# zhangyi-3/UCDIR

Hardware: AMD Instinct MI355X
Metric: restored images/sec at 50-step p_sample_loop, 256x256 SID (higher is better)
Workload: dtype bf16

## Files before the change

### ucdir_amd/csrc/conv_ws128.hip.h

```cpp
#pragma once
#include <type_traits>
#include "conv_ws.hip.h"

struct CvWs128 {
    static constexpr int PITCH = 24;
    static constexpr int PLANE = 10 * PITCH * 128;
    static constexpr int HALO = 2 * PLANE;
    static constexpr int QSTEP = 2 * PITCH * 128;
    static constexpr int OFF_A2 = 2 * HALO;
    static constexpr int A2_BYTES = 2 * 8 * 2 * 32 * 16;
    static constexpr int OFF_TCS = OFF_A2 + A2_BYTES;
    static constexpr int OFF_B2 = OFF_TCS + 9 * 64 * 4;
    static constexpr int OFF_SCAL = OFF_B2 + 64 * 4;
    static constexpr int LDS = OFF_SCAL + 128;
    static constexpr int THREADS = 256;
    static constexpr int DEPTH = 3;
};

__global__ __launch_bounds__(CvWs128::THREADS, 1) void conv_ws128_kernel(const GemmP p) {
    using L = CvWs128;
    extern __shared__ __attribute__((aligned(16))) unsigned char smem[];
    float* const tcs = reinterpret_cast<float*>(smem + L::OFF_TCS);
    float* const b2s = reinterpret_cast<float*>(smem + L::OFF_B2);
    float* const scal = reinterpret_cast<float*>(smem + L::OFF_SCAL);
    const int tid = threadIdx.x, lane = tid & 63, l31 = lane & 31, hh = lane >> 5;
    const int wave = __builtin_amdgcn_readfirstlane(tid >> 6);
    const int rw = wave & 1, pw = wave >> 1;
    const int prow = l31 >> 4, pcol = (l31 & 15) ^ (prow << 3);
    int lid;
    {
        const int nblk = gridDim.x, bid = blockIdx.x;
        const int q = nblk >> 3, r = nblk & 7, xcd = bid & 7;
        lid = (xcd < r ? xcd * (q + 1) : r * (q + 1) + (xcd - r) * q) + (bid >> 3);
    }
#ifdef UCDIR_TIMING
    const bool dbg_on = p.dbg && (lid == (int)gridDim.x / 2 + 3) && (lane == 0) && (wave == 1);
    int dbg_n = 0;
#define C8_STAMP() do { if (dbg_on && dbg_n < 250) p.dbg[dbg_n++] = __builtin_amdgcn_s_memtime(); } while (0)
#else
#define C8_STAMP() do {} while (0)
#endif
    C8_STAMP();
    const int tps = p.tiles_x * p.tiles_y;
    const int T = p.nbatch * tps;
    const int t_beg = (int)((long long)lid * T / (int)gridDim.x), t_end = (int)((long long)(lid + 1) * T / (int)gridDim.x);
    if (t_beg >= t_end) return;

    bf16x8_t af[72];
    {
        const bf16_t* Ab = p.A + ((rw * 72 * 2 + hh) * 32 + l31) * 8;
#pragma unroll
        for (int j = 0; j < 72; ++j) af[j] = *reinterpret_cast<const bf16x8_t*>(Ab + j * (2 * 32 * 8));
    }
#pragma unroll
    for (int j = 0; j < 72; ++j) asm volatile("" : "+v"(af[j]));
    for (int i = tid; i < L::A2_BYTES / 16; i += L::THREADS)
        reinterpret_cast<uint4*>(smem + L::OFF_A2)[i] = reinterpret_cast<const uint4*>(p.alt_A)[i];
    if (tid < 64) b2s[tid] = p.bias2 ? p.bias2[tid] : 0.f;
    __syncthreads();

    unsigned hrel[3];
#pragma unroll
    for (int c3 = 0; c3 < 3; ++c3) {
        const int col = c3 * 8 + (lane >> 3), hp = wave * L::PITCH + col;
        hrel[c3] = col < 18 ? (unsigned)((wave * p.Wp + col) * 64 + (((lane & 7) ^ ((hp >> 1) & 7)) << 3)) * 2u : 0xffffffffu;
    }
    unsigned ba[3][4];
    {
        const int hp0 = (4 * pw + prow) * L::PITCH + pcol;
#pragma unroll
        for (int kx = 0; kx < 3; ++kx) {
            const int sxh = (((hp0 + kx) >> 1) & 7) ^ hh;
#pragma unroll
            for (int k2 = 0; k2 < 4; ++k2) ba[kx][k2] = ((hp0 + kx) << 7) + (((2 * k2) ^ sxh) << 4);
        }
    }
    const unsigned tc_lane = L::OFF_TCS + (32 * rw + 16 * hh) * 4;
    const unsigned b2_lane = L::OFF_B2 + (32 * rw + 16 * hh) * 4;
    const unsigned a2_lane = L::OFF_A2 + ((rw * 8 * 2 + hh) * 32 + l31) * 16;
    const unsigned rel_out = (unsigned)(((4 * pw + prow + 1) * p.Wp + pcol + 1) * 64 + 32 * rw + 16 * hh) * 2;

    int b, ty, tx;
    {
        b = t_beg / tps;
        const int r = t_beg - b * tps;
        ty = r / p.tiles_x; tx = r - ty * p.tiles_x;
    }
    auto issue_tile = [&](int nb, int nty, int ntx, int buf) {
        const long long pix0 = (long long)nty * 8 * p.Wp + ntx * 16;
        const unsigned char* h0 = reinterpret_cast<const unsigned char*>(p.B0 + (long long)nb * p.b0_bstride + pix0 * 64);
        const unsigned char* h1 = reinterpret_cast<const unsigned char*>(p.B1 + (long long)nb * p.b1_bstride + pix0 * 64);
        unsigned char* hd = smem + buf * L::HALO;
        const long long r4 = (long long)4 * p.Wp * 64 * 2;
#pragma unroll
        for (int c3 = 0; c3 < 3; ++c3)
            if (hrel[c3] != 0xffffffffu) {
#pragma unroll
                for (int k = 0; k < 3; ++k)
                    if (k < 2 || wave < 2) {
                        stage16(reinterpret_cast<const bf16_t*>(h0 + k * r4 + hrel[c3]), hd + (3 * (wave + 4 * k) + c3) * 1024, lane);
                        stage16(reinterpret_cast<const bf16_t*>(h1 + k * r4 + hrel[c3]), hd + L::PLANE + (3 * (wave + 4 * k) + c3) * 1024, lane);
                    }
            }
    };
    issue_tile(b, ty, tx, 0);

    int b_cur = -1;
    float rstd_a = 1.f;
    stat_t S1 = 0, S2 = 0;
    const int act = p.act;

#pragma unroll 1
    for (int t = t_beg; t < t_end; ++t) {
        const int buf = (t - t_beg) & 1;
        const bool last = t + 1 == t_end;
        C8_STAMP();
        if (t == t_beg) { HC_WAIT(0); }
        asm volatile("s_barrier" ::: "memory");
        C8_STAMP();
        if (b != b_cur) {
            if (b_cur >= 0 && p.stats_out) {
                const stat_t a = wave_sum_ll(S1), q2 = wave_sum_ll(S2);
                if (lane == 0) stat_add_fx(p.stats_out, b_cur, a, q2);
            }
            S1 = 0; S2 = 0;
            b_cur = b;
            if (wave == 0) {
                float mean = 0.f, rstd = 1.f;
                if (p.fold) {
                    long long v = 0;
                    if (lane < 2 * UCDIR_STAT_SLOTS) {
                        v = p.stats0[(long long)b * (2 * UCDIR_STAT_SLOTS) + lane];
                        if (p.stats1) v += p.stats1[(long long)b * (2 * UCDIR_STAT_SLOTS) + lane];
                    }
#pragma unroll
                    for (int off = 2; off < 2 * UCDIR_STAT_SLOTS; off <<= 1) v += __shfl_xor(v, off);
                    const long long q = __shfl(v, 1);
                    mean_rstd(stat_val(v), stat_val(q), p.inv_count, mean, rstd);
                }
                if (lane == 0) { scal[0] = mean; scal[1] = rstd; }
            }
            __syncthreads();
            const float mean = scal[0], rstd = scal[1];
            for (int i = tid; i < 9 * 64; i += L::THREADS) {
                const int cls = i >> 6, f = i & 63;
                float v = p.bias ? p.bias[f] : 0.f;
                if (p.fold) v += p.Tb[(long long)cls * p.tab_ld + f] - mean * rstd * p.Tg[(long long)cls * p.tab_ld + f];
                tcs[i] = v;
            }
            rstd_a = __builtin_bit_cast(float, __builtin_amdgcn_readfirstlane(__builtin_bit_cast(int, p.alpha * (p.fold ? rstd : 1.0f))));
            __syncthreads();
        }
        int nb = b, nty = ty, ntx = tx + 1;
        if (ntx == p.tiles_x) { ntx = 0; if (++nty == p.tiles_y) { nty = 0; ++nb; } }
        C8_STAMP();

        if (t != t_beg) {
            const int d = buf ? L::HALO : -L::HALO;
#pragma unroll
            for (int kx = 0; kx < 3; ++kx)
#pragma unroll
                for (int k2 = 0; k2 < 4; ++k2) ba[kx][k2] += d;
        }

        f32x16_t acc[2];
        {
            bf16x8_t bq[L::DEPTH + 1][2];
            const long long npix0 = (long long)nty * 8 * p.Wp + ntx * 16;
            const unsigned char* h0 = reinterpret_cast<const unsigned char*>(p.B0 + (long long)nb * p.b0_bstride + npix0 * 64);
            const unsigned char* h1 = reinterpret_cast<const unsigned char*>(p.B1 + (long long)nb * p.b1_bstride + npix0 * 64);
            unsigned char* const hd = smem + (buf ^ 1) * L::HALO;
            const long long r4 = (long long)4 * p.Wp * 64 * 2;
            __builtin_amdgcn_sched_barrier(0);
            asm volatile("s_waitcnt lgkmcnt(0)" ::: "memory");
            static_for<0, L::DEPTH>([&](auto jc) {
                constexpr int j = decltype(jc)::value;
                constexpr int tap = j >> 3, c16 = j & 7, ky = tap / 3, kx = tap - 3 * ky;
                constexpr int off = (c16 >> 2) * L::PLANE + ky * (L::PITCH * 128);
                lds_read16_asm<off>(bq[j][0], ba[kx][(c16 & 3) ^ (ky == 1 ? 2 : 0)]);
                lds_read16_asm<off + L::QSTEP>(bq[j][1], ba[kx][(c16 & 3) ^ (ky == 1 ? 2 : 0)]);
            });
            static_for<0, 72>([&](auto jc) {
                constexpr int j = decltype(jc)::value;
                if constexpr (j + L::DEPTH < 72) {
                    constexpr int jn = j + L::DEPTH;
                    constexpr int tap = jn >> 3, c16 = jn & 7, ky = tap / 3, kx = tap - 3 * ky;
                    constexpr int off = (c16 >> 2) * L::PLANE + ky * (L::PITCH * 128);
                    lds_read16_asm<off>(bq[jn % (L::DEPTH + 1)][0], ba[kx][(c16 & 3) ^ (ky == 1 ? 2 : 0)]);
                    lds_read16_asm<off + L::QSTEP>(bq[jn % (L::DEPTH + 1)][1], ba[kx][(c16 & 3) ^ (ky == 1 ? 2 : 0)]);
                }
                if constexpr (j % 4 == 1 && j / 4 < 18) {
                    constexpr int e = j / 4, c3 = e / 6, k = (e % 6) >> 1, pl = e & 1;
                    if (!last && (k < 2 || wave < 2) && hrel[c3] != 0xffffffffu)
                        stage16(reinterpret_cast<const bf16_t*>((pl ? h1 : h0) + k * r4 + hrel[c3]),
                                hd + pl * L::PLANE + (3 * (wave + 4 * k) + c3) * 1024, lane);
                }
                constexpr int ahead = (71 - j) < L::DEPTH ? (71 - j) : L::DEPTH;
                lgkm_wait_asm<2 * ahead>();
                const f32x16_t zero = {0.f, 0.f, 0.f, 0.f, 0.f, 0.f, 0.f, 0.f, 0.f, 0.f, 0.f, 0.f, 0.f, 0.f, 0.f, 0.f};
                acc[0] = __builtin_amdgcn_mfma_f32_32x32x16_bf16(af[j], bq[j % (L::DEPTH + 1)][0], j ? acc[0] : zero, 0, 0, 0);
                acc[1] = __builtin_amdgcn_mfma_f32_32x32x16_bf16(af[j], bq[j % (L::DEPTH + 1)][1], j ? acc[1] : zero, 0, 0, 0);
            });
            __builtin_amdgcn_sched_barrier(0);
        }
        C8_STAMP();
        f32x16_t acc2[2];
        {
            const f32x16_t zero = {0.f, 0.f, 0.f, 0.f, 0.f, 0.f, 0.f, 0.f, 0.f, 0.f, 0.f, 0.f, 0.f, 0.f, 0.f, 0.f};
#pragma unroll
            for (int j = 0; j < 8; ++j) {
                const bf16x8_t a2 = *reinterpret_cast<const bf16x8_t*>(smem + a2_lane + j * 1024);
                const unsigned a0 = ba[1][(j & 3) ^ 2] + (j >> 2) * L::PLANE + L::PITCH * 128;
                const bf16x8_t b0 = *reinterpret_cast<const bf16x8_t*>(smem + a0);
                const bf16x8_t b1 = *reinterpret_cast<const bf16x8_t*>(smem + a0 + L::QSTEP);
                acc2[0] = __builtin_amdgcn_mfma_f32_32x32x16_bf16(a2, b0, j ? acc2[0] : zero, 0, 0, 0);
                acc2[1] = __builtin_amdgcn_mfma_f32_32x32x16_bf16(a2, b1, j ? acc2[1] : zero, 0, 0, 0);
            }
        }

        C8_STAMP();
        const bool interior = ty > 0 && tx > 0 && ty + 1 < p.tiles_y && tx + 1 < p.tiles_x;
        const long long tile_el = (long long)(ty * 8 * p.Wp + tx * 16) * 64;
        unsigned char* outb = reinterpret_cast<unsigned char*>(reinterpret_cast<bf16_t*>(p.out) + (long long)b * p.out_bstride + tile_el);
        unsigned char* out2b = reinterpret_cast<unsigned char*>(p.out2 + (long long)b * p.out2_bstride + tile_el);
        float s1 = 0.f, s2 = 0.f;
        uint4 pk[2][2], pk2[2][2];
#pragma unroll
        for (int tp = 0; tp < 2; ++tp) {
            unsigned tca = tc_lane + 4 * 256;
            if (!interior) {
                const int r = 4 * pw + 2 * tp + prow, c = pcol;
                const int cy = (ty == 0 && r == 0) ? 0 : ((ty + 1 == p.tiles_y && r == 7) ? 2 : 1);
                const int cx = (tx == 0 && c == 0) ? 0 : ((tx + 1 == p.tiles_x && c == 15) ? 2 : 1);
                tca = tc_lane + (cy * 3 + cx) * 256;
            }
            float v[16], w[16];
#pragma unroll
            for (int g4 = 0; g4 < 4; ++g4) {
                const f32x4_t c4 = *reinterpret_cast<const f32x4_t*>(smem + tca + 16 * g4);
                const f32x4_t d4 = *reinterpret_cast<const f32x4_t*>(smem + b2_lane + 16 * g4);
#pragma unroll
                for (int e = 0; e < 4; ++e) {
                    v[4 * g4 + e] = fmaf(acc[tp][4 * g4 + e], rstd_a, c4[e]);
                    w[4 * g4 + e] = acc2[tp][4 * g4 + e] + d4[e];
                }
            }
            if (act == 1) {
#pragma unroll
                for (int i = 0; i < 16; ++i) v[i] = silu_fast(v[i]);
            } else if (act == 2) {
#pragma unroll
                for (int i = 0; i < 16; ++i) v[i] = fmaxf(0.2f * v[i], v[i]);
            }
#pragma unroll
            for (int i = 0; i < 16; ++i) { s1 += v[i]; s2 += v[i] * v[i]; }
            pk[tp][0] = pack8_bf16(v); pk[tp][1] = pack8_bf16(v + 8);
            pk2[tp][0] = pack8_bf16(w); pk2[tp][1] = pack8_bf16(w + 8);
        }
        C8_STAMP();
        HC_WAIT(0);
        C8_STAMP();
#pragma unroll
        for (int tp = 0; tp < 2; ++tp) {
            const long long o = rel_out + (long long)tp * (2 * p.Wp * 64 * 2);
            *reinterpret_cast<uint4*>(outb + o) = pk[tp][0];
            *reinterpret_cast<uint4*>(outb + o + 16) = pk[tp][1];
            *reinterpret_cast<uint4*>(out2b + o) = pk2[tp][0];
            *reinterpret_cast<uint4*>(out2b + o + 16) = pk2[tp][1];
        }
        S1 += stat_fx((double)s1); S2 += stat_fx((double)s2);
        b = nb; ty = nty; tx = ntx;
    }
#ifdef UCDIR_TIMING
    if (dbg_on) p.dbg[255] = dbg_n;
#endif
    if (p.stats_out) {
        const stat_t a = wave_sum_ll(S1), q2 = wave_sum_ll(S2);
        if (lane == 0) stat_add_fx(p.stats_out, b_cur, a, q2);
    }
}
```

### ucdir_amd/csrc/engine.hip

```cpp
#include <hip/hip_runtime.h>

#include <cmath>
#include <cstdio>
#include <cstring>
#include <map>
#include <mutex>
#include <set>
#include <array>
#include <atomic>
#include <memory>
#include <string>
#include <vector>

#include "../../include/ucdir_hip.h"
#include "cgemm.hip.h"
#include "conv_halo.hip.h"
#include "akgm_halo.hip.h"
#include "akgm_pre.hip.h"
#include "akgm_ws.hip.h"
#include "akgm_ws32.hip.h"
#include "akgm_ws64.hip.h"
#include "conv_ws.hip.h"
#include "conv_sk.hip.h"
#include "conv_ws128.hip.h"
// ... 1244 lines not shown
            fl += 2.0 * 9 * d.cin * d.cout * h * w;
        } else {
            const int h = level_dim(c->Hc, d.level), w = level_dim(c->Wc, d.level);
            if (d.skip_c) { require(!skips.empty(), "skip stack underflow"); x1 = (long)skips.back(); skips.pop_back(); }
            r.h1 = ap.get(h, w, d.cout);
            if (d.cin != d.cout) r.res = ap.get(h, w, d.cout, false);
            r.out = ap.get(h, w, d.cout);
            if (d.attn) r.bo = ap.get(h, w, d.cout);
            r.G = (float*)c->apool.alloc((size_t)B * h * w * 8 * sizeof(float));
            const double hw = (double)h * w;
            fl += 2.0 * 9 * d.cin * d.cout * hw + 2.0 * 9 * d.cout * d.cout * hw;
            if (d.cin != d.cout) fl += 2.0 * d.cin * d.cout * hw;
            fl += 2.0 * hw * (3 * 16 + 72 * 8);
            if (d.attn) {
                if (h * w > maxN) maxN = h * w;
                attC = d.cout;
                fl += 2.0 * d.cout * 3 * d.cout * hw + 2.0 * d.cout * d.cout * hw + 4.0 * hw * hw * d.cout;
            }
            ap.put(r.h1); ap.put(r.res); ap.put(r.bo);
        }
        if (x1 >= 0) ap.put(c->rt[x1].out);
        if (cur >= 0 && !is_skip[cur]) ap.put(c->rt[cur].out);
        cur = (long)li;
        if (d.push_skip) { skips.push_back(li); is_skip[li] = true; }
    }
    fl += 2.0 * 9 * c->cfg.inner_channel * c->cfg.channel_mults[0] * c->cfg.out_channel * c->Hc * c->Wc;
    c->flops = fl * B;
    c->fin_act = Act();
    if (!c->fin_w || env().no_fused_final) c->fin_act = make_act(c->apool, B, c->Hc, c->Wc, c->cfg.inner_channel * c->cfg.channel_mults[0], false);
    if (maxN > 0) alloc_attn(c->apool, c->attn, B, maxN, attC, c->cfg.attn_fp16 != 0);
    c->attw = (float*)c->apool.alloc((size_t)c->nblocks * B * 8 * sizeof(float));
    {
        int maxC = 0;
        for (const auto& d : c->layers) if (d.kind == "block" && d.cout > maxC) maxC = d.cout;
        c->tcbuf = (float*)c->apool.alloc((size_t)B * (9 * 8 * maxC + 2) * sizeof(float), false);
    }
    c->guide_ready = false;
}

static void forward(ucdir_ctx* c, const float* cond, const float* xt, const float* level, float* eps, hipStream_t st) {
    struct ScratchScope { ScratchScope(float* p) { t_splitk = p; } ~ScratchScope() { t_splitk = nullptr; } } scratch_scope(c->splitk);
    c->apool.zero_stats(st);
    require(c->finalized, "weights not finalized");
    require(c->guide_ready, "ucdir_prepare_guide must be called before ucdir_unet_forward");
    const int B = c->B, inner = c->cfg.inner_channel;
    {
        const size_t sm = (size_t)(6 * inner + c->nblocks * 8) * sizeof(float);
        hipLaunchKernelGGL(time_mlp_kernel, dim3(B), dim3(256), sm, st, level, inner, c->mlp_w1, c->mlp_b1, c->mlp_w2,
                           c->mlp_b2, c->tw, c->nblocks, c->attw, B);
        HIPC(hipGetLastError());
    }
    std::vector<const Act*> skips;
    const Act* cur = nullptr;
    for (size_t li = 0; li < c->layers.size(); ++li) {
        const LayerDesc& d = c->layers[li];
        const LayerW& w = c->lw[li];
        LayerRT& r = c->rt[li];
        if (d.kind == "stem") {
            const int tx = (c->Wc + 15) / 16, ty = (c->Hc + 15) / 16;
            const int units = tx * ty * (d.cout / 64) * B;
            hipLaunchKernelGGL((stem_mfma_kernel<6, 0>), dim3(units < 4 * num_cus() ? units : 4 * num_cus()), dim3(256), 0, st, cond, xt, c->H, c->W,
                               c->Hc, c->Wc, d.cout, tx, w.stem_w, r.out.p, r.out.stats, tx * ty, d.cout / 64, B);
            HIPC(hipGetLastError());
        } else if (d.kind == "down") {
            run_conv(w.conv, COLS_DOWN, {*cur, nullptr, r.out, 0, nullptr, true}, st);
        } else if (d.kind == "up") {
            run_conv(w.conv, COLS_UP, {*cur, nullptr, r.out, 0, nullptr, true}, st);
        } else {
            const Act* x0 = cur; const Act* x1 = nullptr;
            if (d.skip_c) { x1 = skips.back(); skips.pop_back(); require(x1->C == d.skip_c, "skip channel mismatch"); }
            const bool res_done = run_conv(w.conv, COLS_S1, {*x0, x1, r.h1, 1, nullptr, true, w.has_res ? &r.res : nullptr, w.has_res ? &w.resconv : nullptr}, st);
            const Act* res = x0;
            if (w.has_res) { if (!res_done) run_conv(w.resconv, COLS_S1, {*x0, x1, r.res, 0, nullptr, false}, st); res = &r.res; }
            Act& bo = d.attn ? r.bo : r.out;
            run_akgm(w.sp, r.h1, r.G, c->attw + (size_t)w.block_index * B * 8, *res, bo, c->tcbuf, st);
            if (d.attn) run_attention(w.qkv, w.outp, bo, r.out, c->attn, st);
        }
        cur = &r.out;
        if (d.push_skip) skips.push_back(cur);
    }
    {
        const int C = cur->C, co = c->cfg.out_channel;
        if (!env().no_fused_final && c->fin_w) {
            const int tiles = ((c->Wc + 15) / 16) * ((c->Hc + 15) / 16) * B;
            const dim3 grid(tiles < 3 * num_cus() ? tiles : 3 * num_cus());
            const size_t lds = (size_t)324 * 80 + (size_t)9 * (C / 32) * 1024 + (size_t)8 * C + (size_t)8 * B;
            require(lds <= 160 * 1024, "final conv: channel count too large for the fused kernel");
            hipLaunchKernelGGL(final_conv_kernel, grid, dim3(256), lds, st, cur->p, c->Hc, c->Wc, C, cur->stats,
                               1.0 / ((double)C * c->Hc * c->Wc), c->fin_gamma, c->fin_beta, c->fin_w, c->fin_b, co, eps, c->H, c->W, B);
            HIPC(hipGetLastError());
        } else {
            hipLaunchKernelGGL(gn_silu_kernel, dim3(2048, 1, B), dim3(256), 0, st, cur->p, c->fin_act.p, c->Hc, c->Wc, C,
                               cur->stats, 1.0 / ((double)C * c->Hc * c->Wc), c->fin_gamma, c->fin_beta);
            HIPC(hipGetLastError());
            Act dummy; dummy.B = B; dummy.H = c->Hc; dummy.W = c->Wc; dummy.C = c->fin_conv.cout;
            run_conv(c->fin_conv, COLS_S1, {c->fin_act, nullptr, dummy, 0, nullptr, false, nullptr, nullptr, eps, c->H, c->W}, st);
        }
    }
}

static void forward_graph(ucdir_ctx* c, const float* cond, const float* xt, const float* level, float* eps, hipStream_t st) {
    for (auto& f : c->graphs)
        if (f.cond == cond && f.xt == xt && f.lvl == level && f.eps == eps) { c->miss_streak = 0; HIPC(hipGraphLaunch(f.ex, st)); return; }
    const bool same_as_last = c->last_miss[0] == cond && c->last_miss[1] == xt && c->last_miss[2] == level && c->last_miss[3] == eps;
    c->last_miss[0] = cond; c->last_miss[1] = xt; c->last_miss[2] = level; c->last_miss[3] = eps;
    if (c->miss_streak >= 2 && !same_as_last) { ++c->miss_streak; forward(c, cond, xt, level, eps, st); return; }
    ++c->miss_streak;
    if (c->graphs.size() >= 8) { const int ms = c->miss_streak; c->drop_graphs(); c->miss_streak = ms; }
    if (!c->cap_stream) HIPC(hipStreamCreateWithFlags(&c->cap_stream, hipStreamNonBlocking));
    HIPC(hipStreamSynchronize(st));
    ucdir_ctx::FwdGraph f{cond, xt, level, eps, nullptr, nullptr};
    HIPC(hipStreamBeginCapture(c->cap_stream, hipStreamCaptureModeThreadLocal));
    try { forward(c, cond, xt, level, eps, c->cap_stream); }
    catch (...) { hipGraph_t g = nullptr; (void)hipStreamEndCapture(c->cap_stream, &g); if (g) (void)hipGraphDestroy(g); throw; }
    HIPC(hipStreamEndCapture(c->cap_stream, &f.g));
    if (hipGraphInstantiate(&f.ex, f.g, nullptr, nullptr, 0) != hipSuccess) {
        (void)hipGraphDestroy(f.g);
        throw std::runtime_error("hipGraphInstantiate failed for a captured forward");
    }
    c->graphs.push_back(f);
    HIPC(hipGraphLaunch(f.ex, st));
}

extern "C" {

int32_t ucdir_abi_version(void) { return UCDIR_ABI_VERSION; }
const char* ucdir_last_error(void) { return g_err.c_str(); }

int32_t ucdir_create(const ucdir_config* cfg, ucdir_ctx** out) {
    API_BEGIN
    require(cfg && out, "null argument");
    require(cfg->n_mults >= 1 && cfg->n_mults <= UCDIR_MAX_MULTS, "bad n_mults");
    require(cfg->inner_channel % 64 == 0, "inner_channel must be a multiple of 64");
    int ndev = 0;
    hipError_t e = hipGetDeviceCount(&ndev);
    require(e == hipSuccess && ndev > 0, "no HIP device available (libucdir_hip has no CPU fallback)");
    require(cfg->device >= 0 && cfg->device < ndev, "bad device ordinal");
    DevGuard dg(cfg->device);
    ensure_kernel_attrs();
    std::unique_ptr<ucdir_ctx> c(new ucdir_ctx());
    c->cfg = *cfg;
    c->layers = build_layers(*cfg);
    for (const auto& d : c->layers)
        if (d.kind == "block") require(d.cout == 64 || d.cout % 128 == 0, "block channels must be 64 or a multiple of 128");
    c->wnames = expected_names(*cfg, c->layers);
    *out = c.release();
    API_END
}

void ucdir_destroy(ucdir_ctx* ctx) {
    if (!ctx) return;
    try { DevGuard dg(ctx->cfg.device); ctx->drop_graphs(); delete ctx; } catch (...) {}
}

int32_t ucdir_num_weights(const ucdir_ctx* ctx) { return ctx ? (int32_t)ctx->wnames.size() : 0; }
const char* ucdir_weight_name(const ucdir_ctx* ctx, int32_t i) {
    if (!ctx || i < 0 || i >= (int32_t)ctx->wnames.size()) return nullptr;
    return ctx->wnames[i].c_str();
}

int32_t ucdir_load_weight(ucdir_ctx* ctx, const char* name, const float* data_host, const int64_t* shape, int32_t ndim) {
    API_BEGIN
    require(ctx && name && data_host && shape, "null argument");
    HostT t; size_t n = 1;
    for (int i = 0; i < ndim; ++i) { t.shape.push_back(shape[i]); n *= (size_t)shape[i]; }
    t.v.assign(data_host, data_host + n);
    ctx->host[name] = std::move(t);
    ctx->finalized = false;
    API_END
// ... 1066 lines not shown
```

### ucdir_amd/csrc/misc.hip.h

```cpp
#pragma once
#include "common.h"

__global__ void act_stats_kernel(const bf16_t* __restrict__ x, int H, int W, int C, stat_t* __restrict__ stats) {
    const int b = blockIdx.x;
    const int Wp = W + 2;
    const long long bs = (long long)(H + 2) * Wp * C;
    const int c8 = C / 8;
    double s1 = 0, s2 = 0;
    for (long long i = threadIdx.x; i < (long long)H * W * c8; i += blockDim.x) {
        int c = (int)(i % c8);
        long long pix = i / c8;
        int y = (int)(pix / W), xx = (int)(pix % W);
        const uint4 v = *reinterpret_cast<const uint4*>(x + b * bs + ((long long)(y + 1) * Wp + xx + 1) * C + c * 8);
        const bf16_t* h = reinterpret_cast<const bf16_t*>(&v);
#pragma unroll
        for (int k = 0; k < 8; ++k) { float f = bf2f(h[k]); s1 += f; s2 += (double)f * f; }
    }
    __shared__ double sh[2][256];
    sh[0][threadIdx.x] = s1; sh[1][threadIdx.x] = s2;
    __syncthreads();
    for (int o = 128; o > 0; o >>= 1) {
        if ((int)threadIdx.x < o) { sh[0][threadIdx.x] += sh[0][threadIdx.x + o]; sh[1][threadIdx.x] += sh[1][threadIdx.x + o]; }
        __syncthreads();
    }
// ... 108 lines not shown
                if (j == 4 && hh) bfr[tp] = __builtin_bit_cast(bf16x8_t, make_uint4(0x3F803F80u, 0u, 0u, 0u));
            }
#pragma unroll
            for (int tm = 0; tm < 2; ++tm)
#pragma unroll
                for (int tp = 0; tp < 2; ++tp)
                    acc[tm][tp] = __builtin_amdgcn_mfma_f32_32x32x16_bf16(af[tm], bfr[tp], acc[tm][tp], 0, 0, 0);
        }
        float s1 = 0.f, s2 = 0.f;
        unsigned char* ot = otile + wv * (32 * 144);
#pragma unroll
        for (int tp = 0; tp < 2; ++tp) {
            {
                const int slot = lane & 31;
                const int y = y0 + wv * 4 + tp * 2 + (slot >> 4), x = x0 + (slot & 15);
                const bool inb = y < Hc && x < Wc;
#pragma unroll
                for (int tm = 0; tm < 2; ++tm)
#pragma unroll
                    for (int g = 0; g < 4; ++g) {
                        const int ch = tm * 32 + 8 * g + 4 * hh;
                        float vv[4] = {acc[tm][tp][4 * g + 0], acc[tm][tp][4 * g + 1], acc[tm][tp][4 * g + 2], acc[tm][tp][4 * g + 3]};
#pragma unroll
                        for (int i = 0; i < 4; ++i) {
                            if (ACT == 2) vv[i] = fmaxf(0.2f * vv[i], vv[i]);
                            if (inb) { s1 += vv[i]; s2 += vv[i] * vv[i]; }
                        }
                        *reinterpret_cast<uint2*>(ot + slot * 144 + ch * 2) = make_uint2(pack2_bf16(vv[0], vv[1]), pack2_bf16(vv[2], vv[3]));
                    }
            }
#pragma unroll
            for (int i = 0; i < 4; ++i) {
                const int idx = i * 64 + lane, slot = idx >> 3, c16 = idx & 7;
                const int y = y0 + wv * 4 + tp * 2 + (slot >> 4), x = x0 + (slot & 15);
                if (y < Hc && x < Wc)
                    *reinterpret_cast<uint4*>(out + (((long long)b * (Hc + 2) + y + 1) * (Wc + 2) + x + 1) * C0 + cb * 64 + c16 * 8) =
                        *reinterpret_cast<const uint4*>(ot + slot * 144 + c16 * 16);
            }
        }
        if (stats_out) {
            for (int off = 32; off > 0; off >>= 1) { s1 += __shfl_xor(s1, off); s2 += __shfl_xor(s2, off); }
            if (lane == 0) { red[wv * 2] = s1; red[wv * 2 + 1] = s2; }
            __syncthreads();
            if (tid == 0) stat_add(stats_out, b, red[0] + red[2] + red[4] + red[6], red[1] + red[3] + red[5] + red[7]);
        }
    }
}

__global__ __launch_bounds__(256) void gn_silu_kernel(const bf16_t* __restrict__ x, bf16_t* __restrict__ y, int H, int W, int C,
                                                      const stat_t* __restrict__ stats, double inv_count,
                                                      const float* __restrict__ gamma, const float* __restrict__ beta) {
    const int b = blockIdx.z;
    float mean, rstd;
    {
        double S, Q;
        stat_read(stats, nullptr, b, S, Q);
        double m = S * inv_count;
        double var = Q * inv_count - m * m;
        if (var < 0) var = 0;
        mean = (float)m; rstd = (float)(1.0 / sqrt(var + 1e-5));
    }
    const int c8n = C / 8;
    const long long bs = (long long)(H + 2) * (W + 2) * C;
    const long long n = (long long)H * W * c8n;
    for (long long i = blockIdx.x * (long long)blockDim.x + threadIdx.x; i < n; i += (long long)gridDim.x * blockDim.x) {
        const int c = (int)(i % c8n) * 8;
        const long long pix = i / c8n;
        const int yy = (int)(pix / W), xx = (int)(pix % W);
        const long long off = b * bs + ((long long)(yy + 1) * (W + 2) + xx + 1) * C + c;
        const uint4 v = *reinterpret_cast<const uint4*>(x + off);
        const bf16_t* h = reinterpret_cast<const bf16_t*>(&v);
        const float4 g0 = *reinterpret_cast<const float4*>(gamma + c), g1 = *reinterpret_cast<const float4*>(gamma + c + 4);
        const float4 b0 = *reinterpret_cast<const float4*>(beta + c), b1 = *reinterpret_cast<const float4*>(beta + c + 4);
        const float gg[8] = {g0.x, g0.y, g0.z, g0.w, g1.x, g1.y, g1.z, g1.w};
        const float bb[8] = {b0.x, b0.y, b0.z, b0.w, b1.x, b1.y, b1.z, b1.w};
        float fv[8];
#pragma unroll
        for (int k = 0; k < 8; ++k) fv[k] = silu_fast((bf2f(h[k]) - mean) * rstd * gg[k] + bb[k]);
        *reinterpret_cast<uint4*>(y + off) = pack8_bf16(fv);
    }
}

typedef __attribute__((ext_vector_type(4))) float f32x4_t;
__global__ __launch_bounds__(256) void final_conv_kernel(const bf16_t* __restrict__ x, int H, int W, int C,
                                                         const stat_t* __restrict__ stats, double inv_count,
                                                         const float* __restrict__ gamma, const float* __restrict__ beta,
                                                         const bf16_t* __restrict__ wfrag, const float* __restrict__ bias, int cout,
                                                         float* __restrict__ out, int crop_h, int crop_w, int nb) {
    extern __shared__ __attribute__((aligned(16))) unsigned char fsm[];
    constexpr int RS = 80;
    unsigned char* wl = fsm + 324 * RS;
    const int nc32 = C / 32, nstep = 9 * nc32;
    for (int it = threadIdx.x; it < nstep * 64; it += 256)
        *reinterpret_cast<uint4*>(wl + it * 16) = *reinterpret_cast<const uint4*>(wfrag + (long long)it * 8);
    float* gb = reinterpret_cast<float*>(wl + nstep * 1024);
    float* ms = gb + 2 * C;
    for (int i = threadIdx.x; i < nb; i += 256) {
        double S, Q;
        float mean, rstd;
        stat_read(stats, nullptr, i, S, Q);
        mean_rstd(S, Q, inv_count, mean, rstd);
        ms[2 * i] = mean; ms[2 * i + 1] = rstd;
    }
    __syncthreads();
    const int lane = threadIdx.x & 63, wv = threadIdx.x >> 6;
    const int col = lane & 15, kg = lane >> 4;
    const int tiles_x = (W + 15) >> 4, tiles_y = (H + 15) >> 4, tps = tiles_x * tiles_y, total = nb * tps;
    int b_cur = -1;
    for (int t = blockIdx.x; t < total; t += gridDim.x) {
        const int b = t / tps, r = t - b * tps, ty = r / tiles_x, tx = r - ty * tiles_x;
        const int x0 = tx * 16, y0 = ty * 16;
        const bf16_t* xb = x + (long long)b * (H + 2) * (W + 2) * C;
        uint4 v[6]; int dst[6]; long long src[6];
#pragma unroll
        for (int u = 0; u < 6; ++u) {
            const int it = threadIdx.x + u * 256;
            dst[u] = -1; src[u] = 0;
            if (it < 324 * 4) {
                const int hp = it >> 2, c = (it & 3) * 8;
                const int hr = hp / 18, hc = hp - hr * 18;
                const int gy = y0 + hr - 1, gx = x0 + hc - 1;
                dst[u] = (hp * RS + c * 2) | ((gy >= 0 && gy < H && gx >= 0 && gx < W) ? 0 : (1 << 30));
                src[u] = ((long long)(gy + 1) * (W + 2) + gx + 1) * C + c;
            }
        }
        auto request = [&](int c32) {
#pragma unroll
            for (int u = 0; u < 6; ++u) {
                v[u] = make_uint4(0, 0, 0, 0);
                if (dst[u] >= 0 && !(dst[u] >> 30)) v[u] = *reinterpret_cast<const uint4*>(xb + src[u] + c32 * 32);
            }
        };
        request(0);
        if (b != b_cur) {
            const float mean = ms[2 * b], rstd = ms[2 * b + 1];
            for (int i = threadIdx.x; i < C; i += 256) { const float sc = rstd * gamma[i]; gb[i] = sc; gb[C + i] = beta[i] - mean * sc; }
            b_cur = b;
        }
        f32x4_t acc[4];
#pragma unroll
        for (int tq = 0; tq < 4; ++tq) acc[tq] = (f32x4_t){0.f, 0.f, 0.f, 0.f};
        for (int c32 = 0; c32 < nc32; ++c32) {
            __syncthreads();
#pragma unroll
            for (int u = 0; u < 6; ++u) {
                if (dst[u] < 0) continue;
                uint4 o = make_uint4(0, 0, 0, 0);
                const int off = dst[u] & ((1 << 30) - 1);
                if (!(dst[u] >> 30)) {
                    const int c = c32 * 32 + ((threadIdx.x + u * 256) & 3) * 8;
                    const bf16_t* h = reinterpret_cast<const bf16_t*>(&v[u]);
                    float fv[8];
#pragma unroll
                    for (int k = 0; k < 8; ++k) fv[k] = silu_fast(fmaf(bf2f(h[k]), gb[c + k], gb[C + c + k]));
                    o = pack8_bf16(fv);
                }
                *reinterpret_cast<uint4*>(fsm + off) = o;
            }
            if (c32 + 1 < nc32) request(c32 + 1);
            __syncthreads();
            for (int tap = 0; tap < 9; ++tap) {
                const int ky = tap / 3, kx = tap - 3 * ky;
                const bf16x8_t af = *reinterpret_cast<const bf16x8_t*>(wl + ((tap * nc32 + c32) * 64 + lane) * 16);
#pragma unroll
                for (int tq = 0; tq < 4; ++tq) {
                    const int hp = (wv * 4 + tq + ky) * 18 + col + kx;
                    const bf16x8_t bf = *reinterpret_cast<const bf16x8_t*>(fsm + hp * RS + kg * 16);
                    acc[tq] = __builtin_amdgcn_mfma_f32_16x16x32_bf16(af, bf, acc[tq], 0, 0, 0);
                }
            }
        }
        if (kg == 0) {
            const int xx = x0 + col;
#pragma unroll
            for (int tq = 0; tq < 4; ++tq) {
                const int y = y0 + wv * 4 + tq;
                if (y < crop_h && xx < crop_w) {
#pragma unroll
                    for (int o = 0; o < 4; ++o)
                        if (o < cout) out[(((long long)b * cout + o) * crop_h + y) * crop_w + xx] = acc[tq][o] + bias[o];
                }
            }
        }
    }
}

__global__ __launch_bounds__(256) void time_mlp_kernel(const float* __restrict__ level, int inner,
                                                       const float* __restrict__ w1, const float* __restrict__ b1,
                                                       const float* __restrict__ w2, const float* __restrict__ b2,
                                                       const float* __restrict__ tw, int nblocks,
                                                       float* __restrict__ attw , int B) {
    extern __shared__ float tsm[];
    float* enc = tsm;
    float* h1 = tsm + inner;
    float* temb = h1 + 4 * inner;
    float* hid = temb + inner;
    const int b = blockIdx.x;
    const float lv = level[b];
    const int half = inner / 2;
    for (int k = threadIdx.x; k < half; k += 256) {
        const float step = (float)k / (float)half;
        const float e = lv * expf(-9.210340371976184f * step);
        enc[k] = sinf(e); enc[k + half] = cosf(e);
    }
    __syncthreads();
    for (int o = threadIdx.x; o < 4 * inner; o += 256) {
        float a = b1[o];
        for (int k = 0; k < inner; ++k) a += w1[o * inner + k] * enc[k];
        h1[o] = a / (1.0f + expf(-a));
    }
    __syncthreads();
    for (int o = threadIdx.x; o < inner; o += 256) {
        float a = b2[o];
        for (int k = 0; k < 4 * inner; ++k) a += w2[o * 4 * inner + k] * h1[k];
        temb[o] = a;
    }
    __syncthreads();
    const int per = 8 * inner + 8 + 64 + 8;
    for (int i = threadIdx.x; i < nblocks * 8; i += 256) {
        const int l = i / 8, o = i % 8;
        const float* W0 = tw + (long long)l * per;
        float a = W0[8 * inner + o];
        for (int k = 0; k < inner; ++k) a += W0[o * inner + k] * temb[k];
        hid[i] = a / (1.0f + expf(-a));
    }
    __syncthreads();
    for (int i = threadIdx.x; i < nblocks * 8; i += 256) {
        const int l = i / 8, o = i % 8;
        const float* W2 = tw + (long long)l * per + 8 * inner + 8;
        float a = W2[64 + o];
        for (int k = 0; k < 8; ++k) a += W2[o * 8 + k] * hid[l * 8 + k];
        attw[((long long)l * B + b) * 8 + o] = a;
    }
}

__global__ __launch_bounds__(256) void guide_branch_kernel(const float* __restrict__ guide, int H, int W, int Hc, int Wc,
                                                           int k, const float* __restrict__ gw, float* __restrict__ G) {
    __shared__ float sw[16 * 3 + 16 + 576 + 8];
    for (int i = threadIdx.x; i < 16 * 3 + 16 + 576 + 8; i += 256) sw[i] = gw[i];
    __syncthreads();
    const float* W0 = sw; const float* b0 = sw + 48; const float* W2 = sw + 64; const float* b2 = sw + 64 + 576;
    const int Hl = Hc / k, Wl = Wc / k;
    const int b = blockIdx.z;
    const int pix = blockIdx.x * 256 + threadIdx.x;
    if (pix >= Hl * Wl) return;
    const int y = pix / Wl, x = pix % Wl;
    float out[8];
#pragma unroll
    for (int o = 0; o < 8; ++o) out[o] = b2[o];
    for (int ky = 0; ky < 3; ++ky) {
        const int yy = y + ky - 1;
        if (yy < 0 || yy >= Hl) continue;
        for (int kx = 0; kx < 3; ++kx) {
            const int xx = x + kx - 1;
            if (xx < 0 || xx >= Wl) continue;
            float g3[3];
#pragma unroll
            for (int c = 0; c < 3; ++c) {
                const float* gp = guide + ((long long)b * 3 + c) * H * W;
                if (k == 1) {
                    g3[c] = gp[(long long)reflect_idx(yy, H) * W + reflect_idx(xx, W)];
                } else {
                    const int y0 = k * yy + k / 2 - 1, x0 = k * xx + k / 2 - 1;
                    const int ya = reflect_idx(y0, H), yb = reflect_idx(y0 + 1, H);
                    const int xa = reflect_idx(x0, W), xb = reflect_idx(x0 + 1, W);
                    const float top = 0.5f * gp[(long long)ya * W + xa] + 0.5f * gp[(long long)ya * W + xb];
// ... 240 lines not shown
```

Baseline: 37.14.

## Fuse secondary 1x1 MFMA chain into pipelined conv loop and pin A fragments to AGPRs

Extends the software-pipelined LDS-read/MFMA loop from 72 to 80 steps so the 8 secondary (alt_A) MFMAs reuse the same depth-3 prefetch pipeline instead of running as a separate unpipelined loop. The lgkmcnt wait counts are computed per step to account for the extra A2 read in the tail steps. Most of the resident A weight fragments are now constrained to AGPRs instead of VGPRs, freeing VGPRs for the extra prefetch buffers. The risk is that AGPR-sourced MFMA operands cost extra moves or add register pressure, and the wait counts must match the actual number of outstanding reads.

```diff
diff --git a/ucdir_amd/csrc/conv_ws128.hip.h b/ucdir_amd/csrc/conv_ws128.hip.h
--- a/ucdir_amd/csrc/conv_ws128.hip.h
+++ b/ucdir_amd/csrc/conv_ws128.hip.h
@@ -15,6 +15,13 @@
     static constexpr int LDS = OFF_SCAL + 128;
     static constexpr int THREADS = 256;
     static constexpr int DEPTH = 3;
+    static constexpr int STEPS = 72 + 8;
+    static constexpr int younger_reads(int j) {
+        int n = 0;
+        for (int s = j + 1; s <= j + DEPTH && s < STEPS; ++s) n += s < 72 ? 2 : 3;
+        return n;
+    }
+    static constexpr int A_VGPR = 24;
 };
 
 __global__ __launch_bounds__(CvWs128::THREADS, 1) void conv_ws128_kernel(const GemmP p) {
@@ -53,7 +60,10 @@
         for (int j = 0; j < 72; ++j) af[j] = *reinterpret_cast<const bf16x8_t*>(Ab + j * (2 * 32 * 8));
     }
 #pragma unroll
-    for (int j = 0; j < 72; ++j) asm volatile("" : "+v"(af[j]));
+    for (int j = 0; j < 72; ++j) {
+        if (j < L::A_VGPR) asm volatile("" : "+v"(af[j]));
+        else asm volatile("" : "+a"(af[j]));
+    }
     for (int i = tid; i < L::A2_BYTES / 16; i += L::THREADS)
         reinterpret_cast<uint4*>(smem + L::OFF_A2)[i] = reinterpret_cast<const uint4*>(p.alt_A)[i];
     if (tid < 64) b2s[tid] = p.bias2 ? p.bias2[tid] : 0.f;
@@ -163,59 +173,46 @@
                 for (int k2 = 0; k2 < 4; ++k2) ba[kx][k2] += d;
         }
 
-        f32x16_t acc[2];
+        f32x16_t acc[2], acc2[2];
         {
-            bf16x8_t bq[L::DEPTH + 1][2];
+            bf16x8_t bq[L::DEPTH + 1][2], aq[L::DEPTH + 1];
             const long long npix0 = (long long)nty * 8 * p.Wp + ntx * 16;
             const unsigned char* h0 = reinterpret_cast<const unsigned char*>(p.B0 + (long long)nb * p.b0_bstride + npix0 * 64);
             const unsigned char* h1 = reinterpret_cast<const unsigned char*>(p.B1 + (long long)nb * p.b1_bstride + npix0 * 64);
             unsigned char* const hd = smem + (buf ^ 1) * L::HALO;
             const long long r4 = (long long)4 * p.Wp * 64 * 2;
+            auto read_step = [&](auto jc) {
+                constexpr int j = decltype(jc)::value, s = j % (L::DEPTH + 1);
+                constexpr int tap = j < 72 ? j >> 3 : 4, c16 = j & 7, ky = tap / 3, kx = tap - 3 * ky;
+                constexpr int off = (c16 >> 2) * L::PLANE + ky * (L::PITCH * 128);
+                if constexpr (j >= 72) lds_read16_asm<(j - 72) * 1024>(aq[s], a2_lane);
+                lds_read16_asm<off>(bq[s][0], ba[kx][(c16 & 3) ^ (ky == 1 ? 2 : 0)]);
+                lds_read16_asm<off + L::QSTEP>(bq[s][1], ba[kx][(c16 & 3) ^ (ky == 1 ? 2 : 0)]);
+            };
             __builtin_amdgcn_sched_barrier(0);
             asm volatile("s_waitcnt lgkmcnt(0)" ::: "memory");
-            static_for<0, L::DEPTH>([&](auto jc) {
-                constexpr int j = decltype(jc)::value;
-                constexpr int tap = j >> 3, c16 = j & 7, ky = tap / 3, kx = tap - 3 * ky;
-                constexpr int off = (c16 >> 2) * L::PLANE + ky * (L::PITCH * 128);
-                lds_read16_asm<off>(bq[j][0], ba[kx][(c16 & 3) ^ (ky == 1 ? 2 : 0)]);
-                lds_read16_asm<off + L::QSTEP>(bq[j][1], ba[kx][(c16 & 3) ^ (ky == 1 ? 2 : 0)]);
-            });
-            static_for<0, 72>([&](auto jc) {
-                constexpr int j = decltype(jc)::value;
-                if constexpr (j + L::DEPTH < 72) {
-                    constexpr int jn = j + L::DEPTH;
-                    constexpr int tap = jn >> 3, c16 = jn & 7, ky = tap / 3, kx = tap - 3 * ky;
-                    constexpr int off = (c16 >> 2) * L::PLANE + ky * (L::PITCH * 128);
-                    lds_read16_asm<off>(bq[jn % (L::DEPTH + 1)][0], ba[kx][(c16 & 3) ^ (ky == 1 ? 2 : 0)]);
-                    lds_read16_asm<off + L::QSTEP>(bq[jn % (L::DEPTH + 1)][1], ba[kx][(c16 & 3) ^ (ky == 1 ? 2 : 0)]);
-                }
+            static_for<0, L::DEPTH>(read_step);
+            static_for<0, L::STEPS>([&](auto jc) {
+                constexpr int j = decltype(jc)::value, s = j % (L::DEPTH + 1);
+                if constexpr (j == 72) C8_STAMP();
+                if constexpr (j + L::DEPTH < L::STEPS) read_step(std::integral_constant<int, j + L::DEPTH>{});
                 if constexpr (j % 4 == 1 && j / 4 < 18) {
                     constexpr int e = j / 4, c3 = e / 6, k = (e % 6) >> 1, pl = e & 1;
                     if (!last && (k < 2 || wave < 2) && hrel[c3] != 0xffffffffu)
                         stage16(reinterpret_cast<const bf16_t*>((pl ? h1 : h0) + k * r4 + hrel[c3]),
                                 hd + pl * L::PLANE + (3 * (wave + 4 * k) + c3) * 1024, lane);
                 }
-                constexpr int ahead = (71 - j) < L::DEPTH ? (71 - j) : L::DEPTH;
-                lgkm_wait_asm<2 * ahead>();
+                lgkm_wait_asm<L::younger_reads(j)>();
                 const f32x16_t zero = {0.f, 0.f, 0.f, 0.f, 0.f, 0.f, 0.f, 0.f, 0.f, 0.f, 0.f, 0.f, 0.f, 0.f, 0.f, 0.f};
-                acc[0] = __builtin_amdgcn_mfma_f32_32x32x16_bf16(af[j], bq[j % (L::DEPTH + 1)][0], j ? acc[0] : zero, 0, 0, 0);
-                acc[1] = __builtin_amdgcn_mfma_f32_32x32x16_bf16(af[j], bq[j % (L::DEPTH + 1)][1], j ? acc[1] : zero, 0, 0, 0);
+                if constexpr (j < 72) {
+                    acc[0] = __builtin_amdgcn_mfma_f32_32x32x16_bf16(af[j], bq[s][0], j ? acc[0] : zero, 0, 0, 0);
+                    acc[1] = __builtin_amdgcn_mfma_f32_32x32x16_bf16(af[j], bq[s][1], j ? acc[1] : zero, 0, 0, 0);
+                } else {
+                    acc2[0] = __builtin_amdgcn_mfma_f32_32x32x16_bf16(aq[s], bq[s][0], j > 72 ? acc2[0] : zero, 0, 0, 0);
+                    acc2[1] = __builtin_amdgcn_mfma_f32_32x32x16_bf16(aq[s], bq[s][1], j > 72 ? acc2[1] : zero, 0, 0, 0);
+                }
             });
             __builtin_amdgcn_sched_barrier(0);
-        }
-        C8_STAMP();
-        f32x16_t acc2[2];
-        {
-            const f32x16_t zero = {0.f, 0.f, 0.f, 0.f, 0.f, 0.f, 0.f, 0.f, 0.f, 0.f, 0.f, 0.f, 0.f, 0.f, 0.f, 0.f};
-#pragma unroll
-            for (int j = 0; j < 8; ++j) {
-                const bf16x8_t a2 = *reinterpret_cast<const bf16x8_t*>(smem + a2_lane + j * 1024);
-                const unsigned a0 = ba[1][(j & 3) ^ 2] + (j >> 2) * L::PLANE + L::PITCH * 128;
-                const bf16x8_t b0 = *reinterpret_cast<const bf16x8_t*>(smem + a0);
-                const bf16x8_t b1 = *reinterpret_cast<const bf16x8_t*>(smem + a0 + L::QSTEP);
-                acc2[0] = __builtin_amdgcn_mfma_f32_32x32x16_bf16(a2, b0, j ? acc2[0] : zero, 0, 0, 0);
-                acc2[1] = __builtin_amdgcn_mfma_f32_32x32x16_bf16(a2, b1, j ? acc2[1] : zero, 0, 0, 0);
-            }
         }
 
         C8_STAMP();
```

After: 37.31, median of 6. About the same (+0.4%).

## Restructure fused final conv: compact weights, crop-only tiles, cross-tile prefetch

Applied to the files above, without the earlier changes.

The fused GN+SiLU+3x3 final conv now stores only the 16 weight fragments per step that hold real output channels (272 bytes instead of 1024). This cuts LDS use so up to four blocks can share a CU, and the grid grows to 4x CUs. Tiles now cover only the cropped output region, and the loop is flattened so the next tile's first channel chunk is prefetched while the current tile finishes. Halo addressing is precomputed as relative offsets with a validity bitmask to save registers and index arithmetic. The trade-off is more complex control flow and a dependence on the persistent grid setting.

```diff
diff --git a/ucdir_amd/csrc/engine.hip b/ucdir_amd/csrc/engine.hip
--- a/ucdir_amd/csrc/engine.hip
+++ b/ucdir_amd/csrc/engine.hip
@@ -1350,9 +1350,11 @@
     {
         const int C = cur->C, co = c->cfg.out_channel;
         if (!env().no_fused_final && c->fin_w) {
-            const int tiles = ((c->Wc + 15) / 16) * ((c->Hc + 15) / 16) * B;
-            const dim3 grid(tiles < 3 * num_cus() ? tiles : 3 * num_cus());
-            const size_t lds = (size_t)324 * 80 + (size_t)9 * (C / 32) * 1024 + (size_t)8 * C + (size_t)8 * B;
+            const int tiles = ((c->W + 15) / 16) * ((c->H + 15) / 16) * B;
+            int G = tiles < 4 * num_cus() ? tiles : 4 * num_cus();
+            if (g_persist_grid > 0 && g_persist_grid < G) G = g_persist_grid;
+            const dim3 grid(G);
+            const size_t lds = (size_t)324 * 80 + (size_t)9 * (C / 32) * 272 + (size_t)8 * C + (size_t)8 * B;
             require(lds <= 160 * 1024, "final conv: channel count too large for the fused kernel");
             hipLaunchKernelGGL(final_conv_kernel, grid, dim3(256), lds, st, cur->p, c->Hc, c->Wc, C, cur->stats,
                                1.0 / ((double)C * c->Hc * c->Wc), c->fin_gamma, c->fin_beta, c->fin_w, c->fin_b, co, eps, c->H, c->W, B);
diff --git a/ucdir_amd/csrc/misc.hip.h b/ucdir_amd/csrc/misc.hip.h
--- a/ucdir_amd/csrc/misc.hip.h
+++ b/ucdir_amd/csrc/misc.hip.h
@@ -214,20 +214,28 @@
 }
 
 typedef __attribute__((ext_vector_type(4))) float f32x4_t;
-__global__ __launch_bounds__(256) void final_conv_kernel(const bf16_t* __restrict__ x, int H, int W, int C,
-                                                         const stat_t* __restrict__ stats, double inv_count,
-                                                         const float* __restrict__ gamma, const float* __restrict__ beta,
-                                                         const bf16_t* __restrict__ wfrag, const float* __restrict__ bias, int cout,
-                                                         float* __restrict__ out, int crop_h, int crop_w, int nb) {
+__global__ __launch_bounds__(256, 4) void final_conv_kernel(const bf16_t* __restrict__ x, int H, int W, int C,
+                                                            const stat_t* __restrict__ stats, double inv_count,
+                                                            const float* __restrict__ gamma, const float* __restrict__ beta,
+                                                            const bf16_t* __restrict__ wfrag, const float* __restrict__ bias, int cout,
+                                                            float* __restrict__ out, int crop_h, int crop_w, int nb) {
     extern __shared__ __attribute__((aligned(16))) unsigned char fsm[];
     constexpr int RS = 80;
-    unsigned char* wl = fsm + 324 * RS;
+    constexpr int ROWB = 18 * RS;
+    constexpr int WS = 17 * 16;
+    unsigned char* wl = fsm + 18 * ROWB;
     const int nc32 = C / 32, nstep = 9 * nc32;
-    for (int it = threadIdx.x; it < nstep * 64; it += 256)
-        *reinterpret_cast<uint4*>(wl + it * 16) = *reinterpret_cast<const uint4*>(wfrag + (long long)it * 8);
-    float* gb = reinterpret_cast<float*>(wl + nstep * 1024);
+    const int tid = threadIdx.x, lane = tid & 63, wv = tid >> 6;
+    const int col = lane & 15, kg = lane >> 4;
+    for (int it = tid; it < nstep * 17; it += 256) {
+        const int step = it / 17, e = it - step * 17;
+        uint4 w = make_uint4(0, 0, 0, 0);
+        if (e < 16) w = *reinterpret_cast<const uint4*>(wfrag + ((long long)step * 64 + (e >> 2) * 16 + (e & 3)) * 8);
+        *reinterpret_cast<uint4*>(wl + it * 16) = w;
+    }
+    float* gb = reinterpret_cast<float*>(wl + nstep * WS);
     float* ms = gb + 2 * C;
-    for (int i = threadIdx.x; i < nb; i += 256) {
+    for (int i = tid; i < nb; i += 256) {
         double S, Q;
         float mean, rstd;
         stat_read(stats, nullptr, i, S, Q);
@@ -235,65 +243,84 @@
         ms[2 * i] = mean; ms[2 * i + 1] = rstd;
     }
     __syncthreads();
-    const int lane = threadIdx.x & 63, wv = threadIdx.x >> 6;
-    const int col = lane & 15, kg = lane >> 4;
-    const int tiles_x = (W + 15) >> 4, tiles_y = (H + 15) >> 4, tps = tiles_x * tiles_y, total = nb * tps;
-    int b_cur = -1;
-    for (int t = blockIdx.x; t < total; t += gridDim.x) {
-        const int b = t / tps, r = t - b * tps, ty = r / tiles_x, tx = r - ty * tiles_x;
-        const int x0 = tx * 16, y0 = ty * 16;
-        const bf16_t* xb = x + (long long)b * (H + 2) * (W + 2) * C;
-        uint4 v[6]; int dst[6]; long long src[6];
+    const int woff = (col < 4 ? kg * 4 + col : 16) * 16;
+    const int c8 = (tid & 3) * 8, dst0 = (tid >> 2) * RS + c8 * 2;
+    const bool last = tid < 324 * 4 - 5 * 256;
+    unsigned rel[6]; int hyp = 0, hxp = 0;
+#pragma unroll
+    for (int u = 0; u < 6; ++u) {
+        const int hp = (tid >> 2) + 64 * u, hr = hp / 18, hc = hp - hr * 18;
+        rel[u] = (unsigned)((hr * (W + 2) + hc) * C + c8) * 2u;
+        hyp |= hr << (5 * u); hxp |= hc << (5 * u);
+    }
+    const int tiles_x = (crop_w + 15) >> 4, tiles_y = (crop_h + 15) >> 4, tps = tiles_x * tiles_y, total = nb * tps;
+    int t = blockIdx.x;
+    if (t >= total) return;
+    int b, x0, y0, vm;
+    const char* xt;
+    auto tile = [&](int tt, int& tb, int& tx0, int& ty0, const char*& txt, int& tvm) {
+        tb = tt / tps;
+        const int r = tt - tb * tps, ty = r / tiles_x;
+        tx0 = (r - ty * tiles_x) * 16; ty0 = ty * 16;
+        txt = reinterpret_cast<const char*>(x + ((long long)tb * (H + 2) * (W + 2) + (long long)ty0 * (W + 2) + tx0) * C);
+        tvm = 0;
 #pragma unroll
         for (int u = 0; u < 6; ++u) {
-            const int it = threadIdx.x + u * 256;
-            dst[u] = -1; src[u] = 0;
-            if (it < 324 * 4) {
-                const int hp = it >> 2, c = (it & 3) * 8;
-                const int hr = hp / 18, hc = hp - hr * 18;
-                const int gy = y0 + hr - 1, gx = x0 + hc - 1;
-                dst[u] = (hp * RS + c * 2) | ((gy >= 0 && gy < H && gx >= 0 && gx < W) ? 0 : (1 << 30));
-                src[u] = ((long long)(gy + 1) * (W + 2) + gx + 1) * C + c;
-            }
-        }
-        auto request = [&](int c32) {
-#pragma unroll
-            for (int u = 0; u < 6; ++u) {
-                v[u] = make_uint4(0, 0, 0, 0);
-                if (dst[u] >= 0 && !(dst[u] >> 30)) v[u] = *reinterpret_cast<const uint4*>(xb + src[u] + c32 * 32);
-            }
-        };
-        request(0);
-        if (b != b_cur) {
-            const float mean = ms[2 * b], rstd = ms[2 * b + 1];
-            for (int i = threadIdx.x; i < C; i += 256) { const float sc = rstd * gamma[i]; gb[i] = sc; gb[C + i] = beta[i] - mean * sc; }
-            b_cur = b;
-        }
-        f32x4_t acc[4];
-#pragma unroll
-        for (int tq = 0; tq < 4; ++tq) acc[tq] = (f32x4_t){0.f, 0.f, 0.f, 0.f};
-        for (int c32 = 0; c32 < nc32; ++c32) {
-            __syncthreads();
-#pragma unroll
-            for (int u = 0; u < 6; ++u) {
-                if (dst[u] < 0) continue;
-                uint4 o = make_uint4(0, 0, 0, 0);
-                const int off = dst[u] & ((1 << 30) - 1);
-                if (!(dst[u] >> 30)) {
-                    const int c = c32 * 32 + ((threadIdx.x + u * 256) & 3) * 8;
-                    const bf16_t* h = reinterpret_cast<const bf16_t*>(&v[u]);
-                    float fv[8];
-#pragma unroll
-                    for (int k = 0; k < 8; ++k) fv[k] = silu_fast(fmaf(bf2f(h[k]), gb[c + k], gb[C + c + k]));
-                    o = pack8_bf16(fv);
-                }
-                *reinterpret_cast<uint4*>(fsm + off) = o;
-            }
-            if (c32 + 1 < nc32) request(c32 + 1);
-            __syncthreads();
-            for (int tap = 0; tap < 9; ++tap) {
-                const int ky = tap / 3, kx = tap - 3 * ky;
-                const bf16x8_t af = *reinterpret_cast<const bf16x8_t*>(wl + ((tap * nc32 + c32) * 64 + lane) * 16);
+            const int gy = ty0 + ((hyp >> (5 * u)) & 31) - 1, gx = tx0 + ((hxp >> (5 * u)) & 31) - 1;
+            if ((u < 5 || last) && gy >= 0 && gy < H && gx >= 0 && gx < W) tvm |= 1 << u;
+        }
+    };
+    uint4 v[6];
+    auto request = [&](const char* xp, int m) {
+#pragma unroll
+        for (int u = 0; u < 6; ++u) v[u] = *reinterpret_cast<const uint4*>(xp + (((m >> u) & 1) ? rel[u] : 0u));
+    };
+    tile(t, b, x0, y0, xt, vm);
+    request(xt, vm);
+    int b_cur = -1, c32 = 0;
+    f32x4_t acc[4];
+    for (;;) {
+        if (c32 == 0) {
+            if (b != b_cur) {
+                const float mean = ms[2 * b], rstd = ms[2 * b + 1];
+                for (int i = tid; i < C; i += 256) { const float sc = rstd * gamma[i]; gb[i] = sc; gb[C + i] = beta[i] - mean * sc; }
+                b_cur = b;
+            }
+#pragma unroll
+            for (int tq = 0; tq < 4; ++tq) acc[tq] = (f32x4_t){0.f, 0.f, 0.f, 0.f};
+        }
+        __syncthreads();
+#pragma unroll
+        for (int u = 0; u < 6; ++u) {
+            if (u == 5 && !last) continue;
+            asm volatile("" : "+v"(v[u].x), "+v"(v[u].y), "+v"(v[u].z), "+v"(v[u].w));
+            uint4 o = make_uint4(0, 0, 0, 0);
+            if ((vm >> u) & 1) {
+                const int c = c32 * 32 + c8;
+                const bf16_t* h = reinterpret_cast<const bf16_t*>(&v[u]);
+                float fv[8];
+#pragma unroll
+                for (int k = 0; k < 8; ++k) fv[k] = silu_fast(fmaf(bf2f(h[k]), gb[c + k], gb[C + c + k]));
+                o = pack8_bf16(fv);
+            }
+            *reinterpret_cast<uint4*>(fsm + dst0 + 64 * RS * u) = o;
+        }
+        const bool done = c32 + 1 == nc32;
+        int tn = t, bn = b, xn = x0, yn = y0, vmn = vm, cn = c32 + 1;
+        const char* xtn = xt;
+        if (done) {
+            tn = t + gridDim.x; cn = 0;
+            if (tn < total) tile(tn, bn, xn, yn, xtn, vmn);
+            else cn = c32;
+        }
+        request(xtn + cn * 64, vmn);
+        __syncthreads();
+#pragma unroll 1
+        for (int ky = 0; ky < 3; ++ky) {
+#pragma unroll
+            for (int kx = 0; kx < 3; ++kx) {
+                const int tap = ky * 3 + kx;
+                const bf16x8_t af = *reinterpret_cast<const bf16x8_t*>(wl + (tap * nc32 + c32) * WS + woff);
 #pragma unroll
                 for (int tq = 0; tq < 4; ++tq) {
                     const int hp = (wv * 4 + tq + ky) * 18 + col + kx;
@@ -302,18 +329,22 @@
                 }
             }
         }
-        if (kg == 0) {
-            const int xx = x0 + col;
-#pragma unroll
-            for (int tq = 0; tq < 4; ++tq) {
-                const int y = y0 + wv * 4 + tq;
-                if (y < crop_h && xx < crop_w) {
-#pragma unroll
-                    for (int o = 0; o < 4; ++o)
-                        if (o < cout) out[(((long long)b * cout + o) * crop_h + y) * crop_w + xx] = acc[tq][o] + bias[o];
+        if (done) {
+            if (kg == 0) {
+                const int xx = x0 + col;
+#pragma unroll
+                for (int tq = 0; tq < 4; ++tq) {
+                    const int y = y0 + wv * 4 + tq;
+                    if (y < crop_h && xx < crop_w) {
+#pragma unroll
+                        for (int o = 0; o < 4; ++o)
+                            if (o < cout) out[(((long long)b * cout + o) * crop_h + y) * crop_w + xx] = acc[tq][o] + bias[o];
+                    }
                 }
             }
-        }
+            if (tn >= total) break;
+        }
+        t = tn; b = bn; x0 = xn; y0 = yn; xt = xtn; vm = vmn; c32 = cn;
     }
 }
 
```

New measurement: 38.40 before, 38.52 after, median of 6. About the same (+0.3%).
